# HKPolyU-UAV/ReinforcementLearningPlatform

Hardware: NVIDIA B200
Metric: env-steps/sec (higher is better)
Workload: dtype f64

## Files before the change

### reinforcementlearningplatform_b200/csrc/common.cuh

```cuda
#pragma once
#include <cuda_runtime.h>
#include <stdint.h>
#include <math.h>
#include "../../include/b200env.h"
#include "fastmath64.cuh"

#define B200_BLOCK 128

template <typename T> struct Mth;

template <> struct Mth<double> {
#ifdef B200_LIBDEVICE_MATH
    static __device__ __forceinline__ void sincos(double x, double *s, double *c) { ::sincos(x, s, c); }
    static __device__ __forceinline__ void sincos3(double a, double b, double c, double *sa, double *ca, double *sb,
                                                   double *cb, double *sc, double *cc) {
        ::sincos(a, sa, ca); ::sincos(b, sb, cb); ::sincos(c, sc, cc);
    }
    static __device__ __forceinline__ void sincos2(double a, double b, double *sa, double *ca, double *sb, double *cb) {
        ::sincos(a, sa, ca); ::sincos(b, sb, cb);
    }
    static __device__ __forceinline__ double rcp(double y) { return 1.0 / y; }
    static __device__ __forceinline__ double div(double x, double y) { return x / y; }
    static __device__ __forceinline__ double tanh(double x) { return ::tanh(x); }
    static __device__ __forceinline__ double log(double x) { return ::log(x); }
    static __device__ __forceinline__ double log_nonneg(double x) { return ::log(x); }
    static __device__ __forceinline__ double exp(double x) { return ::exp(x); }
    static __device__ __forceinline__ double asin(double x) { return ::asin(x); }
#else
    static __device__ __forceinline__ void sincos(double x, double *s, double *c) { fm64::sincos(x, s, c); }
    static __device__ __forceinline__ void sincos3(double a, double b, double c, double *sa, double *ca, double *sb,
                                                   double *cb, double *sc, double *cc) {
        fm64::sincos3(a, b, c, sa, ca, sb, cb, sc, cc);
    }
    static __device__ __forceinline__ void sincos2(double a, double b, double *sa, double *ca, double *sb, double *cb) {
        fm64::sincos2(a, b, sa, ca, sb, cb);
    }
    static __device__ __forceinline__ double rcp(double y) { return fm64::rcp(y); }
    static __device__ __forceinline__ double div(double x, double y) { return fm64::div(x, y); }
    static __device__ __forceinline__ double tanh(double x) { return fm64::tanh(x); }
    static __device__ __forceinline__ double log(double x) { return fm64::log(x); }
    static __device__ __forceinline__ double log_nonneg(double x) { return fm64::log_nonneg(x); }
    static __device__ __forceinline__ double exp(double x) { return fm64::exp(x); }
    static __device__ __forceinline__ double asin(double x) { return fm64::asin(x); }
#endif
#ifndef B200_LIBDEVICE_MATH
    static __device__ __forceinline__ double sin(double x) { double s, c; fm64::sincos(x, &s, &c); return s; }
    static __device__ __forceinline__ double cos(double x) { double s, c; fm64::sincos(x, &s, &c); return c; }
#else
    static __device__ __forceinline__ double sin(double x) { return ::sin(x); }
    static __device__ __forceinline__ double cos(double x) { return ::cos(x); }
#endif
    static __device__ __forceinline__ double sin_ld(double x) { return ::sin(x); }
    static __device__ __forceinline__ double tan(double x) { return ::tan(x); }
    static __device__ __forceinline__ double pow(double x, double y) { return ::pow(x, y); }
    static __device__ __forceinline__ double sqrt(double x) { return ::sqrt(x); }
    static __device__ __forceinline__ double acos(double x) { return ::acos(x); }
    static __device__ __forceinline__ double atan2(double y, double x) { return ::atan2(y, x); }
    static __device__ __forceinline__ double abs(double x) { return ::fabs(x); }
    static __device__ __forceinline__ double min(double a, double b) { return ::fmin(a, b); }
    static __device__ __forceinline__ double max(double a, double b) { return ::fmax(a, b); }
    static __device__ __forceinline__ double fma(double a, double b, double c) { return ::fma(a, b, c); }
};

template <> struct Mth<float> {
    static __device__ __forceinline__ float sin(float x) { return ::sinf(x); }
    static __device__ __forceinline__ float sin_ld(float x) { return ::sinf(x); }
    static __device__ __forceinline__ float cos(float x) { return ::cosf(x); }
    static __device__ __forceinline__ void sincos(float x, float *s, float *c) { ::sincosf(x, s, c); }
    static __device__ __forceinline__ void sincos3(float a, float b, float c, float *sa, float *ca, float *sb, float *cb,
                                                   float *sc, float *cc) {
        ::sincosf(a, sa, ca); ::sincosf(b, sb, cb); ::sincosf(c, sc, cc);
    }
    static __device__ __forceinline__ void sincos2(float a, float b, float *sa, float *ca, float *sb, float *cb) {
        ::sincosf(a, sa, ca); ::sincosf(b, sb, cb);
    }
    static __device__ __forceinline__ float rcp(float y) { return 1.0f / y; }
    static __device__ __forceinline__ float div(float x, float y) { return x / y; }
    static __device__ __forceinline__ float tan(float x) { return ::tanf(x); }
    static __device__ __forceinline__ float tanh(float x) { return ::tanhf(x); }
    static __device__ __forceinline__ float pow(float x, float y) { return ::powf(x, y); }
    static __device__ __forceinline__ float log(float x) { return ::logf(x); }
    static __device__ __forceinline__ float log_nonneg(float x) { return ::logf(x); }
    static __device__ __forceinline__ float exp(float x) { return ::expf(x); }
    static __device__ __forceinline__ float sqrt(float x) { return ::sqrtf(x); }
    static __device__ __forceinline__ float asin(float x) { return ::asinf(x); }
    static __device__ __forceinline__ float acos(float x) { return ::acosf(x); }
    static __device__ __forceinline__ float atan2(float y, float x) { return ::atan2f(y, x); }
    static __device__ __forceinline__ float abs(float x) { return ::fabsf(x); }
    static __device__ __forceinline__ float min(float a, float b) { return ::fminf(a, b); }
    static __device__ __forceinline__ float max(float a, float b) { return ::fmaxf(a, b); }
    static __device__ __forceinline__ float fma(float a, float b, float c) { return ::fmaf(a, b, c); }
};

template <typename T>
__device__ __forceinline__ T pow_from_log(T L, T a) {
    const T r = Mth<T>::exp(a * L);
    return a == (T)0 ? (T)1 : r;
}

#ifndef B200_SOA_INDEX
template <typename T, bool IO32, typename I>
__device__ __forceinline__ T ldio(const void *base, I n, int field, I i) {
    constexpr int ES = IO32 ? 4 : (int)sizeof(T);
    const char *p = static_cast<const char *>(base) + (uint64_t)(uint32_t)i * ES + (uint64_t)(uint32_t)n * (uint32_t)(field * ES);
    if (IO32) return (T) * reinterpret_cast<const float *>(p);
    return *reinterpret_cast<const T *>(p);
}
template <typename T, bool IO32, typename I>
__device__ __forceinline__ void stio(void *base, I n, int field, I i, T v) {
    constexpr int ES = IO32 ? 4 : (int)sizeof(T);
    char *p = static_cast<char *>(base) + (uint64_t)(uint32_t)i * ES + (uint64_t)(uint32_t)n * (uint32_t)(field * ES);
    if (IO32) *reinterpret_cast<float *>(p) = (float)v;
    else *reinterpret_cast<T *>(p) = v;
}
#else
template <typename T, bool IO32, typename I>
__device__ __forceinline__ T ldio(const void *base, I n, int field, I i) {
    if (IO32) return (T) static_cast<const float *>(base)[(I)field * n + i];
    return static_cast<const T *>(base)[(I)field * n + i];
}
template <typename T, bool IO32, typename I>
__device__ __forceinline__ void stio(void *base, I n, int field, I i, T v) {
    if (IO32) static_cast<float *>(base)[(I)field * n + i] = (float)v;
    else static_cast<T *>(base)[(I)field * n + i] = v;
}
#endif

template <typename T, bool IO32, typename I>
__device__ __forceinline__ T ldio_idx(const void *base, I n, int field, I i) {
    if (IO32) return (T) static_cast<const float *>(base)[(I)field * n + i];
    return static_cast<const T *>(base)[(I)field * n + i];
}
template <typename T, bool IO32, typename I>
__device__ __forceinline__ void stio_idx(void *base, I n, int field, I i, T v) {
    if (IO32) static_cast<float *>(base)[(I)field * n + i] = (float)v;
    else static_cast<T *>(base)[(I)field * n + i] = v;
}

template <typename T>
__device__ __forceinline__ T np_norm2(T a, T b) { return Mth<T>::sqrt(Mth<T>::fma(b, b, a * a)); }

__device__ __forceinline__ double mul_rn(double a, double b) { return __dmul_rn(a, b); }
__device__ __forceinline__ float mul_rn(float a, float b) { return __fmul_rn(a, b); }
__device__ __forceinline__ double add_rn(double a, double b) { return __dadd_rn(a, b); }
__device__ __forceinline__ float add_rn(float a, float b) { return __fadd_rn(a, b); }
template <typename T>
__device__ __forceinline__ T sumsq_rn(T a, T b) { return add_rn(mul_rn(a, a), mul_rn(b, b)); }
template <typename T>
__device__ __forceinline__ T sumsq_rn(T a, T b, T c, T d) {
    return add_rn(add_rn(sumsq_rn(a, b), mul_rn(c, c)), mul_rn(d, d));
}

template <typename T>
__device__ __forceinline__ T clampc(T x, T lo, T hi) {
    x = x < lo ? lo : x;
    return x > hi ? hi : x;
}

// ... 138 lines not shown
```

### reinforcementlearningplatform_b200/csrc/fastmath64.cuh

```cuda
#pragma once
#include <cuda_runtime.h>
#include <math.h>
#include <math_constants.h>
#include <stdint.h>

namespace fm64 {

static __constant__ double kS[6] = {-0x1.5555555555555p-3, 0x1.1111111110b23p-7, -0x1.a01a019e623afp-13,
                                    0x1.71de376b9c575p-19, -0x1.ae5fdeb852566p-26, 0x1.5dfb4dfaf15abp-33};
static __constant__ double kC[6] = {0x1.5555555555555p-5, -0x1.6c16c16c1691fp-10, 0x1.a01a019f3df42p-16,
                                    -0x1.27e4fa025e03dp-22, 0x1.1eeb52bea9072p-29, -0x1.906dd38cb66a1p-37};
static __constant__ double kE[10] = {0x1.0000000000001p-1, 0x1.5555555555556p-3, 0x1.5555555553b6cp-5,
                                     0x1.1111111110918p-7, 0x1.6c16c1794e1dcp-10, 0x1.a01a01a83ba17p-13,
                                     0x1.a019b621f9d08p-16, 0x1.71de0be2b5e96p-19, 0x1.2894f52583578p-22,
                                     0x1.af3ce42b12b24p-26};
static __constant__ double kL[7] = {0x1.5555555555558p-1, 0x1.99999999949c3p-2, 0x1.2492492ef134dp-2,
                                    0x1.c71c61a265960p-3, 0x1.74630fb47b087p-3, 0x1.39f2ac8e848c3p-3,
                                    0x1.2be78035f90e7p-3};
static __constant__ double kA[12] = {0x1.555555555554fp-3, 0x1.3333333336f25p-4, 0x1.6db6db682abf8p-5,
                                     0x1.f1c71fa66977fp-6, 0x1.6e8b28e7f8608p-6, 0x1.1c596afc9d8acp-6,
                                     0x1.c86de3215c77bp-7, 0x1.8546aebb901aap-7, 0x1.fdf3b5f7fbfb1p-8,
                                     0x1.07d821fcdce60p-6, -0x1.64309bd35e9c9p-7, 0x1.cf09bf99f54b7p-6};
static __constant__ double kR[8] = {0x1.921fb54442d18p+0, 0x1.1a62633145c07p-54, -0x1.f1976b7ed8fbcp-110,
                                    0x1.45f306dc9c883p-1, 0x1.62e42fefa39efp-1, 0x1.abc9e3b39803fp-56,
                                    0x1.71547652b82fep+0, 6755399441055744.0};

__device__ __forceinline__ double rcp(double y) {
    double r;
    asm("rcp.approx.ftz.f64 %0, %1;" : "=d"(r) : "d"(y));
    double e = fma(-y, r, 1.0);
    r = fma(r, e, r);
    e = fma(-y, r, 1.0);
    r = fma(r, e, r);
    return r;
}
__device__ __forceinline__ double div(double x, double y) {
    const double r = rcp(y);
    const double q = x * r;
    return fma(fma(-y, q, x), r, q);
}

__device__ __forceinline__ double sqrt_nb(double x) {
    double y;
    asm("rsqrt.approx.ftz.f64 %0, %1;" : "=d"(y) : "d"(x));
    double g = x * y, h = 0.5 * y;
    double r = fma(-g, h, 0.5);
    g = fma(g, r, g);
    h = fma(h, r, h);
    r = fma(-g, h, 0.5);
    g = fma(g, r, g);
    h = fma(h, r, h);
    g = fma(fma(-g, g, x), h, g);
    return (x == 0.0 || x == CUDART_INF) ? x : g;
}

__device__ __forceinline__ void sincos_core(double x, double *sn, double *cs) {
    const double t = fma(x, kR[3], kR[7]);
    const int n = __double2loint(t);
    const double fn = t - kR[7];
    double r = fma(-fn, kR[0], x);
    r = fma(-fn, kR[1], r);
    r = fma(-fn, kR[2], r);
    const double z = r * r;
    double ps = kS[5];
    ps = fma(ps, z, kS[4]); ps = fma(ps, z, kS[3]); ps = fma(ps, z, kS[2]); ps = fma(ps, z, kS[1]); ps = fma(ps, z, kS[0]);
    ps = fma(r * z, ps, r);
    double pc = kC[5];
    pc = fma(pc, z, kC[4]); pc = fma(pc, z, kC[3]); pc = fma(pc, z, kC[2]); pc = fma(pc, z, kC[1]); pc = fma(pc, z, kC[0]);
    pc = fma(z, fma(z, pc, -0.5), 1.0);
    const double s = (n & 1) ? pc : ps;
    const double c = (n & 1) ? ps : pc;
    *sn = __hiloint2double(__double2hiint(s) ^ ((n & 2) << 30), __double2loint(s));
    *cs = __hiloint2double(__double2hiint(c) ^ (((n + 1) & 2) << 30), __double2loint(c));
}

__device__ __forceinline__ void sincos(double x, double *sn, double *cs) {
    if (!(fabs(x) < 1.0e5)) {
        ::sincos(x, sn, cs);
        return;
    }
    sincos_core(x, sn, cs);
}

__device__ __forceinline__ void sincos3(double a, double b, double c, double *sa, double *ca, double *sb, double *cb,
                                        double *sc, double *cc) {
    if (!(fabs(a) + fabs(b) + fabs(c) < 1.0e5)) {
        ::sincos(a, sa, ca);
        ::sincos(b, sb, cb);
        ::sincos(c, sc, cc);
        return;
    }
    sincos_core(a, sa, ca);
    sincos_core(b, sb, cb);
    sincos_core(c, sc, cc);
}
__device__ __forceinline__ void sincos2(double a, double b, double *sa, double *ca, double *sb, double *cb) {
    if (!(fabs(a) + fabs(b) < 1.0e5)) {
        ::sincos(a, sa, ca);
        ::sincos(b, sb, cb);
        return;
    }
    sincos_core(a, sa, ca);
    sincos_core(b, sb, cb);
}

__device__ __forceinline__ double exp_core(double x) {
    const double t = fma(x, kR[6], kR[7]);
    const int n = __double2loint(t);
    const double fn = t - kR[7];
    double r = fma(-fn, kR[4], x);
    r = fma(-fn, kR[5], r);
    const double r2 = r * r;
    double pe = kE[8], po = kE[9];
    pe = fma(pe, r2, kE[6]); po = fma(po, r2, kE[7]);
    pe = fma(pe, r2, kE[4]); po = fma(po, r2, kE[5]);
    pe = fma(pe, r2, kE[2]); po = fma(po, r2, kE[3]);
    pe = fma(pe, r2, kE[0]); po = fma(po, r2, kE[1]);
    const double p = fma(po, r, pe);
    const double y = fma(r2, p, r) + 1.0;
    return y * __hiloint2double((n + 1023) << 20, 0);
}

__device__ __forceinline__ double exp(double x) {
    double y = exp_core(x);
    if (x < -708.0) y = 0.0;
    if (x > 709.0) y = CUDART_INF;
    return y;
}

__device__ __forceinline__ double log(double x) {
    int hi = __double2hiint(x);
    const int lo = __double2loint(x);
    int k = (hi >> 20) - 1023;
    hi &= 0x000fffff;
    const int i = (hi + 0x95f64) & 0x100000;
    k += i >> 20;
    const double m = __hiloint2double(hi | (i ^ 0x3ff00000), lo);
    const double f = m - 1.0;
    const double s = div(f, 2.0 + f);
    const double z = s * s;
    double R = kL[6];
    R = fma(R, z, kL[5]); R = fma(R, z, kL[4]); R = fma(R, z, kL[3]); R = fma(R, z, kL[2]); R = fma(R, z, kL[1]);
    R = fma(R, z, kL[0]);
    R *= z;
    const double hfsq = 0.5 * f * f;
    const double dk = (double)k;
    double y = dk * kR[4] - ((hfsq - (s * (hfsq + R) + dk * kR[5])) - f);
    if (x < 2.2250738585072014e-308) y = -CUDART_INF;
    if (!(x >= 0.0)) y = CUDART_NAN;
    if (x == CUDART_INF) y = x;
    return y;
}

__device__ __forceinline__ double log_nonneg(double x) {
    int hi = __double2hiint(x);
    const int lo = __double2loint(x);
    int k = (hi >> 20) - 1023;
    hi &= 0x000fffff;
    const int i = (hi + 0x95f64) & 0x100000;
    k += i >> 20;
    const double m = __hiloint2double(hi | (i ^ 0x3ff00000), lo);
    const double f = m - 1.0;
    const double s = div(f, 2.0 + f);
    const double z = s * s;
    double R = kL[6];
    R = fma(R, z, kL[5]); R = fma(R, z, kL[4]); R = fma(R, z, kL[3]); R = fma(R, z, kL[2]); R = fma(R, z, kL[1]);
    R = fma(R, z, kL[0]);
    R *= z;
    const double hfsq = 0.5 * f * f;
    const double dk = (double)k;
    const double y = dk * kR[4] - ((hfsq - (s * (hfsq + R) + dk * kR[5])) - f);
    return x < 2.2250738585072014e-308 ? -CUDART_INF : y;
}

__device__ __forceinline__ double tanh(double x) {
    const double ax = (fabs(x) > 20.0) ? 20.0 : fabs(x);
    const double t = exp_core(2.0 * ax);
    const double y = fma(-2.0, rcp(t + 1.0), 1.0);
    return copysign(y, x);
}

__device__ __forceinline__ double asin(double x) {
    const double ax = fabs(x);
    const bool big = ax > 0.5;
    const double w = big ? 0.5 * (1.0 - ax) : ax * ax;
    const double t = big ? sqrt_nb(w) : ax;
// ... 11 lines not shown
```

### reinforcementlearningplatform_b200/csrc/uav.cu

```cuda
#include "common.cuh"
#ifndef UAV_POS_MINBLOCKS
#define UAV_POS_MINBLOCKS 4
#endif
#ifndef UAV_ATT_MINBLOCKS
#define UAV_ATT_MINBLOCKS 5
#endif
#include "uav_common.cuh"

namespace {
using namespace uavk;

template <typename T>
__device__ __forceinline__ int terminal_flag(const P &p, const T *x, double time) {
    int flag = 0;
    bool out = false;
#pragma unroll
    for (int i = 0; i < 3; ++i) out = out || (x[i] < (T)p.pos_lo[i]) || (x[i] > (T)p.pos_hi[i]);
    if (out) flag = 2;
    out = false;
#pragma unroll
    for (int i = 0; i < 3; ++i) out = out || (x[6 + i] < (T)p.att_lo[i]) || (x[6 + i] > (T)p.att_hi[i]);
    if (out) flag = 3;
    if (time > p.t_term) flag = 1;
    return flag;
// ... 156 lines not shown
    }
}

template <typename T, bool IO32>
__global__ void __launch_bounds__(B200_BLOCK)
uav_att_reset_kernel(const __grid_constant__ P p, const __grid_constant__ b200env_io io, int64_t n,
                     const uint8_t *mask, uint64_t seed, int64_t off, int observe_only) {
    const int64_t i = (int64_t)blockIdx.x * blockDim.x + threadIdx.x;
    if (i >= n) return;
    if (!observe_only && mask && !mask[i]) return;
    T x[12];
    if (observe_only) {
#pragma unroll
        for (int k = 0; k < 6; ++k) { x[k] = (T)0; x[6 + k] = UAV_LDS(io.state, n, k, i); }
    } else {
        att_reset_state<T, int64_t>(p, io, n, i, seed, off, x);
    }
    if (io.next_obs) {
        T ref[3], dref[3], o[6];
#pragma unroll
        for (int k = 0; k < 3; ++k) { ref[k] = UAV_LDS(io.state, n, A_REF + k, i); dref[k] = UAV_LDS(io.state, n, A_DREF + k, i); }
        Trig<T> t;
        t.eval(x[6], x[7], x[8], false);
        att_observe<T>(x, t, ref, dref, o);
#pragma unroll
        for (int k = 0; k < 6; ++k) stio<T, IO32>(io.next_obs, n, k, i, o[k]);
    }
}

enum { P_SIG = 12, P_S1 = 15, P_AREF = 18, P_K1 = 21, P_K2 = 24, P_GAM = 27, P_LMD = 30, P_AMP = 33, P_PER = 37,
       P_PHS = 41, P_PREF = 45, P_DPREF = 48, P_NEXT_PQR0 = 51  };

template <typename T, typename I>
__device__ __forceinline__ void pos_reset_state(const P &p, const b200env_io &io, I n, I i, uint64_t seed,
                                               int64_t off, T *x) {
    const uint32_t ep = io.episode[i];
#pragma unroll
    for (int k = 0; k < 12; ++k) { x[k] = (T)p.init_state[k]; UAV_STS(io.state, n, k, i, x[k]); }
#pragma unroll
    for (int k = 0; k < 3; ++k) {
        UAV_STS(io.state, n, P_SIG + k, i, (T)0);
        UAV_STS(io.state, n, P_S1 + k, i, (T)0);
        UAV_STS(io.state, n, P_K1 + k, i, (T)p.pos_k1[k]);
        UAV_STS(io.state, n, P_K2 + k, i, (T)p.pos_k2[k]);
        UAV_STS(io.state, n, P_GAM + k, i, (T)p.pos_gamma[k]);
        UAV_STS(io.state, n, P_LMD + k, i, (T)p.pos_lmd[k]);
    }
    double A[4], Tp[4], ph[4];
    Philox rng(seed, (uint64_t)(off + (int64_t)i), ep);
    if (p.random_trajectory) {
        const double a = rng.uniform(0., p.traj_A_hi[0]);
        const double tt = rng.uniform(p.traj_T_lo, p.traj_T_hi);
        A[0] = A[1] = A[2] = a; A[3] = 0.;
#pragma unroll
        for (int k = 0; k < 4; ++k) { Tp[k] = tt; ph[k] = p.ref_bias_phase[k]; }
    } else {
#pragma unroll
        for (int k = 0; k < 4; ++k) { A[k] = p.ref_amplitude[k]; Tp[k] = p.ref_period[k]; ph[k] = p.ref_bias_phase[k]; }
    }
    if (p.yaw_fixed) { A[3] = 0.; ph[3] = 0.; }
#pragma unroll
    for (int k = 0; k < 4; ++k) {
        UAV_STS(io.state, n, P_AMP + k, i, (T)A[k]);
        UAV_STS(io.state, n, P_PER + k, i, (T)Tp[k]);
        UAV_STS(io.state, n, P_PHS + k, i, (T)ph[k]);
    }
    if (p.random_pos0) {
#pragma unroll
        for (int k = 0; k < 3; ++k) {
            const double t0 = p.ref_bias_a[k] + A[k] * ::sin(ph[k]);
            const double r = ::fabs(p.init_pos_r[k]);
            const double pos0 = rng.uniform(t0 - r, t0 + r);
            x[k] = (T)pos0;
            x[9 + k] = UAV_LDS(io.state, n, P_NEXT_PQR0 + k, i);
            UAV_STS(io.state, n, k, i, x[k]);
            UAV_STS(io.state, n, 9 + k, i, x[9 + k]);
            UAV_STS(io.state, n, P_NEXT_PQR0 + k, i, x[k]);
        }
    }
    io.time[i] = 0.0;
    io.episode[i] = ep + 1u;
}

template <typename T, typename I, bool IO32>
__device__ __forceinline__ void uav_pos_step_one(const P &p, const Consts<T> &c, const b200env_io &io, I n, I i,
                                                 uint32_t flags, uint64_t seed, int64_t off) {
    T x[12];
#pragma unroll
    for (int k = 0; k < 12; ++k) x[k] = UAV_LDS(io.state, n, k, i);
    double time = io.time[i];
    T a[8], dis[3] = {(T)0, (T)0, (T)0};
#pragma unroll
    for (int k = 0; k < 8; ++k) a[k] = ldio<T, IO32>(io.action, n, k, i);
    if (io.dis) {
#pragma unroll
        for (int k = 0; k < 3; ++k) dis[k] = ldio<T, IO32>(io.dis, n, k, i);
    }
    T sig[3], s1[3], aref0, aref1, rA[4], rT[4], rP[4];
#pragma unroll
    for (int k = 0; k < 3; ++k) { sig[k] = UAV_LDS(io.state, n, P_SIG + k, i); s1[k] = UAV_LDS(io.state, n, P_S1 + k, i); }
    aref0 = UAV_LDS(io.state, n, P_AREF + 0, i);
    aref1 = UAV_LDS(io.state, n, P_AREF + 1, i);
#pragma unroll
    for (int k = 0; k < 4; ++k) {
        rA[k] = UAV_LDS(io.state, n, P_AMP + k, i); rT[k] = UAV_LDS(io.state, n, P_PER + k, i); rP[k] = UAV_LDS(io.state, n, P_PHS + k, i);
    }
    T k1[3], k2[3], gam[3], lmd[3];
#pragma unroll
    for (int k = 0; k < 3; ++k) {
        k1[k] = a[k] > (T)0 ? a[k] : UAV_LDS(io.state, n, P_K1 + k, i);
        k2[k] = a[k + 3] > (T)0 ? a[k + 3] : UAV_LDS(io.state, n, P_K2 + k, i);
        gam[k] = a[6] > (T)0 ? a[6] : UAV_LDS(io.state, n, P_GAM + k, i);
        lmd[k] = a[7] > (T)0 ? a[7] : UAV_LDS(io.state, n, P_LMD + k, i);
        UAV_STS(io.state, n, P_K1 + k, i, k1[k]);
        UAV_STS(io.state, n, P_K2 + k, i, k2[k]);
        UAV_STS(io.state, n, P_GAM + k, i, gam[k]);
        UAV_STS(io.state, n, P_LMD + k, i, lmd[k]);
    }
    T ref[4], dref[4], ddref[4];
    {
        const T bias4[4] = {(T)p.ref_bias_a[0], (T)p.ref_bias_a[1], (T)p.ref_bias_a[2], (T)p.ref_bias_a[3]};
        ref_channels<T, 4>((T)time, rA, rT, bias4, rP, ref, dref, ddref);
    }
    T ctrl[3];
    const T kt_m = c.kt_m;
#pragma unroll
    for (int k = 0; k < 3; ++k) {
        const T e = x[k] - ref[k], de = x[3 + k] - dref[k];
        T so, dso1, pa1_de;
        smc_axis<T>(e, de, k1[k], gam[k], (T)p.pos_alpha[k], (T)p.pos_beta[k], lmd[k], c.dt, sig[k], so, dso1, pa1_de);
        UAV_STS(io.state, n, P_SIG + k, i, sig[k]);
        const T uo1 = kt_m * x[3 + k] + ddref[k] - k1[k] * de - pa1_de - lmd[k] * dso1;
        const T uo2 = -k2[k] * so;
        ctrl[k] = uo1 + uo2;
    }
    const T u_acc = -(ctrl[0] * ctrl[0] * (T)p.R[0] + ctrl[1] * ctrl[1] * (T)p.R[1] + ctrl[2] * ctrl[2] * (T)p.R[2]);
    Trig<T> t1;
    t1.eval(x[6], x[7], x[8], true);
    const T uf = (ctrl[2] + c.g) * c.m / (t1.cphi * t1.cth);
    const T asin_phi_d = clampc<T>(Mth<T>::div((ctrl[0] * t1.spsi - ctrl[1] * t1.cpsi) * c.m, uf), (T)-1, (T)1);
    T phi_d = Mth<T>::asin(asin_phi_d);
    const T asin_theta_d = clampc<T>(
        Mth<T>::div((ctrl[0] * t1.cpsi + ctrl[1] * t1.spsi) * c.m, uf * cos_of_asin<T>(asin_phi_d, phi_d)), (T)-1, (T)1);
    T theta_d = Mth<T>::asin(asin_theta_d);
    const T lim = (T)p.att_limit;
    phi_d = clampc<T>(phi_d, -lim, lim);
    theta_d = clampc<T>(theta_d, -lim, lim);
    T rho_d[3] = {phi_d, theta_d, ref[3]};
#ifdef B200_STRICT_DIV
    T drho_d[3] = {(phi_d - aref0) / c.dt, (theta_d - aref1) / c.dt, dref[3]};
#else
    const Divisor<T> by_dt(c.dt);
    T drho_d[3] = {by_dt.div(phi_d - aref0), by_dt.div(theta_d - aref1), dref[3]};
#endif
    const T rl = (T)p.dot_att_ref_limit;
#pragma unroll
    for (int k = 0; k < 3; ++k) {
        drho_d[k] = clampc<T>(drho_d[k], -rl, rl);
        rho_d[k] = rho_d[k] + drho_d[k] * c.dt;
        UAV_STS(io.state, n, P_AREF + k, i, rho_d[k]);
    }
    T torque[3], d1[3], ak1[3], ak2[3], agam[3], almd[3], aalpha[3], abeta[3];
#pragma unroll
    for (int k = 0; k < 3; ++k) {
        ak1[k] = (T)p.att_k1[k]; ak2[k] = (T)p.att_k2[k]; agam[k] = (T)p.att_gamma[k]; almd[k] = (T)p.att_lmd[k];
        aalpha[k] = (T)p.att_alpha[k]; abeta[k] = (T)p.att_beta[k];
    }
    att_control<T>(c, x, t1, ak1, ak2, agam, almd, aalpha, abeta, s1, rho_d, drho_d, torque, d1);
#pragma unroll
    for (int k = 0; k < 3; ++k) UAV_STS(io.state, n, P_S1 + k, i, s1[k]);
    if (io.obs) {
#pragma unroll
        for (int k = 0; k < 3; ++k) {
            stio<T, IO32>(io.obs, n, k, i, x[k] - ref[k]);
            stio<T, IO32>(io.obs, n, 3 + k, i, x[3 + k] - dref[k]);
        }
    }
    uav_rk44<T, false>(c, x, t1, uf, torque, dis);
    time += p.dt;
    const int flag = terminal_flag<T>(p, x, time);
    const bool done = flag != 0;
    T nxt[6];
#pragma unroll
    for (int k = 0; k < 3; ++k) { nxt[k] = x[k] - ref[k]; nxt[3 + k] = x[3 + k] - dref[k]; }
    const T u_pos = -(nxt[0] * nxt[0] * (T)p.Q_e[0] + nxt[1] * nxt[1] * (T)p.Q_e[1] + nxt[2] * nxt[2] * (T)p.Q_e[2]);
    const T u_vel = -(nxt[3] * nxt[3] * (T)p.Q_de[0] + nxt[4] * nxt[4] * (T)p.Q_de[1] + nxt[5] * nxt[5] * (T)p.Q_de[2]);
    T u_extra = (T)0;
    if (flag == 2 || flag == 3) {
        const T nn = (T)((p.time_max - time) / p.dt);
        u_extra = nn * (u_pos + u_vel + u_acc);
    }
    const T reward = u_pos + u_vel + u_acc + u_extra;
#pragma unroll
    for (int k = 0; k < 6; ++k) stio<T, IO32>(io.next_obs, n, k, i, nxt[k]);
    stio<T, IO32>(io.reward, n, 0, i, reward);
    io.done[i] = done ? 1 : 0;
    io.flag[i] = flag;
    if (done && (flags & B200ENV_AUTO_RESET)) {
        T xr[12];
        pos_reset_state<T, I>(p, io, n, i, seed, off, xr);
#pragma unroll
        for (int k = 0; k < 3; ++k) { nxt[k] = xr[k] - ref[k]; nxt[3 + k] = xr[3 + k] - dref[k]; }
    } else {
#pragma unroll
        for (int k = 0; k < 12; ++k) UAV_STS(io.state, n, k, i, x[k]);
        io.time[i] = time;
        if (done) {
#pragma unroll
            for (int k = 0; k < 3; ++k) { UAV_STS(io.state, n, P_PREF + k, i, ref[k]); UAV_STS(io.state, n, P_DPREF + k, i, dref[k]); }
        }
    }
    if (io.reset_obs) {
#pragma unroll
        for (int k = 0; k < 6; ++k) stio<T, IO32>(io.reset_obs, n, k, i, nxt[k]);
    }
}

template <typename T, typename I, bool IO32>
__global__ void __launch_bounds__(B200_BLOCK, UAV_POS_MINBLOCKS)
uav_pos_step_kernel(const __grid_constant__ P p, const __grid_constant__ UavDerived dv,
                    const __grid_constant__ b200env_io io, int64_t n_, uint32_t flags, uint64_t seed, int64_t off) {
    const int64_t gi = (int64_t)blockIdx.x * blockDim.x + threadIdx.x;
    if (gi >= n_) return;
    const Consts<T> c(p.m, p.g, p.J, p.kr, p.kt, p.dt, dv);
    uav_pos_step_one<T, I, IO32>(p, c, io, (I)n_, (I)gi, flags, seed, off);
}

template <typename T, bool IO32>
__global__ void __launch_bounds__(B200_BLOCK)
uav_pos_reset_kernel(const __grid_constant__ P p, const __grid_constant__ b200env_io io, int64_t n,
                     const uint8_t *mask, uint64_t seed, int64_t off, int observe_only) {
    const int64_t i = (int64_t)blockIdx.x * blockDim.x + threadIdx.x;
    if (i >= n) return;
    if (!observe_only && mask && !mask[i]) return;
    T x[12];
    if (observe_only) {
#pragma unroll
        for (int k = 0; k < 12; ++k) x[k] = UAV_LDS(io.state, n, k, i);
    } else {
        pos_reset_state<T, int64_t>(p, io, n, i, seed, off, x);
    }
    if (io.next_obs) {
#pragma unroll
        for (int k = 0; k < 3; ++k) {
            stio<T, IO32>(io.next_obs, n, k, i, x[k] - UAV_LDS(io.state, n, P_PREF + k, i));
            stio<T, IO32>(io.next_obs, n, 3 + k, i, x[3 + k] - UAV_LDS(io.state, n, P_DPREF + k, i));
        }
    }
}

}

#define UAV_LAUNCH(kern, ...) B200_LAUNCH_TIO(kern, b200_grid(n), B200_BLOCK, s, __VA_ARGS__)

#define UAV_LAUNCH_STEP(kern, fields, gridexpr, ...)                                                                        \
    do {                                                                                                           \
        const bool i32 = (int64_t)(fields) * n < ((int64_t)1 << 32);                                               \
        const bool o32 = b200_io32(io);                                                                            \
        const unsigned g = (gridexpr);                                                                             \
        if (dtype == B200ENV_F64) {                                                                                \
            if (i32 && o32) kern<double, uint32_t, true><<<g, B200_BLOCK, 0, s>>>(__VA_ARGS__);                    \
            else if (i32) kern<double, uint32_t, false><<<g, B200_BLOCK, 0, s>>>(__VA_ARGS__);                     \
            else if (o32) kern<double, int64_t, true><<<g, B200_BLOCK, 0, s>>>(__VA_ARGS__);                       \
            else kern<double, int64_t, false><<<g, B200_BLOCK, 0, s>>>(__VA_ARGS__);                               \
        } else {                                                                                                   \
            if (i32) kern<float, uint32_t, false><<<g, B200_BLOCK, 0, s>>>(__VA_ARGS__);                           \
            else kern<float, int64_t, false><<<g, B200_BLOCK, 0, s>>>(__VA_ARGS__);                                \
        }                                                                                                          \
    } while (0)

int uav_att_dims(int variant, int *sf, int *od, int *ad, int *dd) {
    if (variant != 0) return B200ENV_EENV;
    if (sf) *sf = B200_UAV_ATT_STATE_FIELDS;
    if (od) *od = 6;
    if (ad) *ad = 8;
    if (dd) *dd = 0;
    return B200ENV_OK;
}
int uav_pos_dims(int variant, int *sf, int *od, int *ad, int *dd) {
    if (variant != 0 && variant != 1) return B200ENV_EENV;
    if (sf) *sf = variant == 1 ? B200_UAV_POS_STATE_FIELDS_V1 : B200_UAV_POS_STATE_FIELDS;
    if (od) *od = 6;
    if (ad) *ad = 8;
    if (dd) *dd = 3;
    return B200ENV_OK;
}

static int uav_check_step(const b200env_io *io, uint32_t flags) {
    if (!io->state || !io->time || !io->action || !io->next_obs || !io->reward || !io->done || !io->flag) return B200ENV_ENULL;
    if ((flags & B200ENV_AUTO_RESET) && !io->episode) return B200ENV_ENULL;
    return B200ENV_OK;
}

int uav_att_step(int dtype, int64_t n, const void *params, const b200env_io *io, uint32_t flags, uint64_t seed,
                 int64_t off, cudaStream_t s) {
    int rc = uav_check_step(io, flags);
    if (rc) return rc;
    const P &p = *static_cast<const P *>(params);
    UAV_LAUNCH_STEP(uav_att_step_kernel, B200_UAV_ATT_STATE_FIELDS, b200_grid(n), p, uav_derive(p.m, p.J, p.kt), *io, n, flags, seed, off);
    return b200_check_launch();
}
int uav_pos_step(int dtype, int64_t n, const void *params, const b200env_io *io, uint32_t flags, uint64_t seed,
                 int64_t off, cudaStream_t s) {
    int rc = uav_check_step(io, flags);
    if (rc) return rc;
    const P &p = *static_cast<const P *>(params);
    UAV_LAUNCH_STEP(uav_pos_step_kernel, B200_UAV_POS_STATE_FIELDS_V1, b200_grid(n), p, uav_derive(p.m, p.J, p.kt), *io, n, flags, seed, off);
    return b200_check_launch();
// ... 28 lines not shown
```

### reinforcementlearningplatform_b200/csrc/uav_common.cuh

```cuda
#pragma once
#include "common.cuh"

#ifdef B200_STRICT
#define B200_STRICT_POW
#define B200_STRICT_TAN
#define B200_STRICT_DIV
#ifndef B200_UAV_LAPACK_INV
#define B200_UAV_LAPACK_INV
#endif
#endif
#ifdef B200_STRICT_DIV
#define UAV_DIV(a, b, rb) ((a) / (b))
#else
#define UAV_DIV(a, b, rb) ((a) * (rb))
#endif

template <typename T, typename I>
__device__ __forceinline__ const char *uav_blk_base(const void *base, I i) {
    return static_cast<const char *>(base) +
           (uint64_t)((uint32_t)i >> 7) * (uint64_t)(B200_UAV_STATE_SLOTS * 128 * sizeof(T)) +
           ((uint32_t)i & 127u) * (uint32_t)sizeof(T);
}
#define UAV_LDS(base, n, field, i) (*reinterpret_cast<const T *>(uav_blk_base<T>(base, i) + (field) * (int)(128 * sizeof(T))))
#define UAV_STS(base, n, field, i, v) (*reinterpret_cast<T *>(const_cast<char *>(uav_blk_base<T>(base, i)) + (field) * (int)(128 * sizeof(T))) = (v))

namespace uavk {

typedef b200_uav_params P;



template <typename T>
struct Trig {
    T sphi, cphi, sth, cth, spsi, cpsi, tth, rcth;
    __device__ __forceinline__ void eval(T phi, T th, T psi, bool need_psi) {
        if (need_psi) {
            Mth<T>::sincos3(phi, th, psi, &sphi, &cphi, &sth, &cth, &spsi, &cpsi);
        } else {
            Mth<T>::sincos2(phi, th, &sphi, &cphi, &sth, &cth);
            spsi = (T)0; cpsi = (T)1;
        }
        rcth = Mth<T>::rcp(cth);
#ifdef B200_STRICT_TAN
        tth = Mth<T>::tan(th);
#else
        tth = sth * rcth;
#endif
    }
};

struct UavDerived {
    double rJ[3], rm, kt_m, J21, J02, J10;
};
static inline UavDerived uav_derive(double m, const double *J, double kt) {
    UavDerived d;
    for (int k = 0; k < 3; ++k) d.rJ[k] = 1.0 / J[k];
    d.rm = 1.0 / m;
    d.kt_m = kt / m;
    d.J21 = J[2] - J[1]; d.J02 = J[0] - J[2]; d.J10 = J[1] - J[0];
    return d;
}

template <typename T>
struct Consts {
    T m, g, kr, kt, J0, J1, J2, J21, J02, J10, dt, rJ0, rJ1, rJ2, rm, kt_m;
    __device__ __forceinline__ Consts(double m_, double g_, const double *J, double kr_, double kt_, double dt_,
                                      const UavDerived &d)
        : m((T)m_), g((T)g_), kr((T)kr_), kt((T)kt_), J0((T)J[0]), J1((T)J[1]), J2((T)J[2]), J21((T)d.J21),
          J02((T)d.J02), J10((T)d.J10), dt((T)dt_), rJ0((T)d.rJ[0]), rJ1((T)d.rJ[1]), rJ2((T)d.rJ[2]), rm((T)d.rm),
          kt_m((T)d.kt_m) {}
};

template <typename T, bool ATT_ONLY>
__device__ __forceinline__ void uav_ode(const Consts<T> &c, const T *x, const Trig<T> &t, T throttle, const T *tq,
                                        const T *dis, T *d) {
    const T p = x[9], q = x[10], r = x[11];
    d[9] = UAV_DIV(-c.kr * p - q * r * c.J21 + tq[0], c.J0, c.rJ0);
    d[10] = UAV_DIV(-c.kr * q - p * r * c.J02 + tq[1], c.J1, c.rJ1);
    d[11] = UAV_DIV(-c.kr * r - p * q * c.J10 + tq[2], c.J2, c.rJ2);
    d[6] = p + (t.tth * t.sphi) * q + (t.tth * t.cphi) * r;
    d[7] = t.cphi * q - t.sphi * r;
    d[8] = UAV_DIV(t.sphi, t.cth, t.rcth) * q + UAV_DIV(t.cphi, t.cth, t.rcth) * r;
    if (!ATT_ONLY) {
        d[0] = x[3]; d[1] = x[4]; d[2] = x[5];
        d[3] = UAV_DIV(throttle * (t.cpsi * t.sth * t.cphi + t.spsi * t.sphi) - c.kt * x[3] + dis[0], c.m, c.rm);
        d[4] = UAV_DIV(throttle * (t.spsi * t.sth * t.cphi - t.cpsi * t.sphi) - c.kt * x[4] + dis[1], c.m, c.rm);
        d[5] = -c.g + UAV_DIV(throttle * t.cphi * t.cth - c.kt * x[5] + dis[2], c.m, c.rm);
    }
}

template <typename T, bool ATT_ONLY>
__device__ __forceinline__ void uav_rk44(const Consts<T> &c, T *x, Trig<T> t, T throttle, const T *tq, const T *dis) {
    constexpr int LO = ATT_ONLY ? 6 : 0;
    const T h = c.dt;
    T acc[12], xs[12];
#pragma unroll
    for (int i = LO; i < 12; ++i) { acc[i] = (T)0; xs[i] = x[i]; }
#pragma unroll 1
    for (int s = 0; s < 4; ++s) {
        T d[12];
        uav_ode<T, ATT_ONLY>(c, xs, t, throttle, tq, dis, d);
        const T w = (s == 0 || s == 3) ? (T)1 : (T)2;
        const T cs = (s == 2) ? (T)1 : (T)0.5;
#pragma unroll
        for (int i = LO; i < 12; ++i) {
            const T k = h * d[i];
            acc[i] = acc[i] + w * k;
            xs[i] = x[i] + k * cs;
        }
        if (s < 3) t.eval(xs[6], xs[7], xs[8], !ATT_ONLY);
    }
#pragma unroll
    for (int i = LO; i < 12; ++i) x[i] = x[i] + UAV_DIV(acc[i], (T)6, (T)(1.0 / 6.0));
    if (x[8] > (T)M_PI) x[8] -= (T)(2 * M_PI);
    if (x[8] < (T)-M_PI) x[8] += (T)(2 * M_PI);
}

template <typename T>
__device__ __forceinline__ void smc_axis(T e, T de, T k1, T gamma, T alpha, T beta, T lmd, T dt, T &integ,
                                         T &s_out, T &dot_s1, T &pa1_de) {
    const T ae = Mth<T>::abs(e);
#ifdef B200_STRICT_POW
    const T s_ = de + k1 * e + gamma * Mth<T>::pow(ae, alpha) * Mth<T>::tanh((T)5 * e);
    dot_s1 = Mth<T>::pow(Mth<T>::abs(s_), beta) * Mth<T>::tanh((T)5 * s_);
    integ += dot_s1 * dt;
    s_out = s_ + lmd * integ;
    pa1_de = gamma * alpha * Mth<T>::pow(ae, alpha - (T)1) * de;
    return;
#endif
    const T L = Mth<T>::log_nonneg(ae);
    const T pa1 = pow_from_log<T>(L, alpha - (T)1);
    const T pa_ = pa1 * ae;
    const T pa = alpha == (T)0 ? (T)1 : ((ae == (T)0 && alpha > (T)0) ? (T)0 : pa_);
    const T s = de + k1 * e + gamma * pa * Mth<T>::tanh((T)5 * e);
    dot_s1 = pow_from_log<T>(Mth<T>::log_nonneg(Mth<T>::abs(s)), beta) * Mth<T>::tanh((T)5 * s);
    integ += dot_s1 * dt;
    s_out = s + lmd * integ;
    pa1_de = gamma * alpha * pa1 * de;
}

template <typename T>
__device__ __forceinline__ void neg_inv_apply(T b00, T b01, T b02, T b11, T b12, T b21, T b22, const T *v, T *out) {
    const bool swap = Mth<T>::abs(b21) > Mth<T>::abs(b11);
    const T u11 = swap ? b21 : b11, u12 = swap ? b22 : b12;
    const T r21 = swap ? b11 : b21, r22 = swap ? b12 : b22;
    const T l = r21 * ((T)1 / u11);
    const T u22 = r22 - l * u12;
    T inv[3][3];
#pragma unroll
    for (int cidx = 0; cidx < 3; ++cidx) {
        T y0 = cidx == 0 ? (T)1 : (T)0;
        T y1 = (cidx == (swap ? 2 : 1)) ? (T)1 : (T)0;
        T y2 = (cidx == (swap ? 1 : 2)) ? (T)1 : (T)0;
        y2 = y2 - l * y1;
        const T x2 = y2 / u22;
        const T x1 = (y1 - u12 * x2) / u11;
        const T x0 = ((y0 - b01 * x1) - b02 * x2) / b00;
        inv[0][cidx] = x0; inv[1][cidx] = x1; inv[2][cidx] = x2;
    }
#pragma unroll
    for (int i = 0; i < 3; ++i) out[i] = -(inv[i][0] * v[0] + inv[i][1] * v[1] + inv[i][2] * v[2]);
}

template <typename T>
__device__ __forceinline__ void att_control(const Consts<T> &c, const T *x, const Trig<T> &t, const T *k1, const T *k2,
                                            const T *gamma, const T *lmd, const T *alpha, const T *beta, T *s1,
                                            const T *ref, const T *dref, T *torque, T *d1) {
    const T p = x[9], q = x[10], r = x[11];
    const T f01 = t.sphi * t.tth, f02 = t.cphi * t.tth, f11 = t.cphi, f12 = -t.sphi;
    const T f21 = UAV_DIV(t.sphi, t.cth, t.rcth), f22 = UAV_DIV(t.cphi, t.cth, t.rcth);
    d1[0] = p + f01 * q + f02 * r;
    d1[1] = f11 * q + f12 * r;
    d1[2] = f21 * q + f22 * r;
    const T rc2 = t.rcth * t.rcth;
    const T c2 = t.cth * t.cth;
    (void)c2;
    const T F01 = d1[0] * t.tth * t.cphi + UAV_DIV(d1[1] * t.sphi, c2, rc2);
    const T F02 = -d1[0] * t.tth * t.sphi + UAV_DIV(d1[1] * t.cphi, c2, rc2);
    const T F11 = -d1[0] * t.sphi, F12 = -d1[0] * t.cphi;
    const T F21 = UAV_DIV(d1[0] * t.cphi * t.cth + d1[1] * t.sphi * t.sth, c2, rc2);
    const T F22 = UAV_DIV(-d1[0] * t.sphi * t.cth + d1[1] * t.cphi * t.sth, c2, rc2);
    const T g0 = UAV_DIV(c.kr * p + q * r * (c.J1 - c.J2), c.J0, c.rJ0);
    const T g1 = UAV_DIV(c.kr * q + p * r * (c.J2 - c.J0), c.J1, c.rJ1);
    const T g2 = UAV_DIV(c.kr * r + p * q * (c.J0 - c.J1), c.J2, c.rJ2);
    T sec[3];
    sec[0] = (F01 * q + F02 * r) + (g0 + f01 * g1 + f02 * g2);
    sec[1] = (F11 * q + F12 * r) + (f11 * g1 + f12 * g2);
    sec[2] = (F21 * q + F22 * r) + (f21 * g1 + f22 * g2);
    T v[3];
#pragma unroll
    for (int i = 0; i < 3; ++i) {
        const T e = x[6 + i] - ref[i], de = d1[i] - dref[i];
        T sigma, dot_s1, pa1_de;
        smc_axis<T>(e, de, k1[i], gamma[i], alpha[i], beta[i], lmd[i], c.dt, s1[i], sigma, dot_s1, pa1_de);
        const T u1 = sec[i] + k1[i] * de + pa1_de + lmd[i] * dot_s1;
        const T u2 = -k2[i] * Mth<T>::tanh((T)10 * sigma);
        v[i] = u1 + u2;
    }
#ifdef B200_UAV_LAPACK_INV
    neg_inv_apply<T>(c.rJ0, f01 * c.rJ1, f02 * c.rJ2, f11 * c.rJ1, f12 * c.rJ2, f21 * c.rJ1, f22 * c.rJ2, v, torque);
#else
    torque[0] = -c.J0 * (v[0] - t.sth * v[2]);
    torque[1] = -c.J1 * (t.cphi * v[1] + t.sphi * t.cth * v[2]);
    torque[2] = -c.J2 * (t.cphi * t.cth * v[2] - t.sphi * v[1]);
#endif
}


template <typename T>
__device__ __forceinline__ T cos_of_asin(T u, T phi_d) {
    if (sizeof(T) == 4) return Mth<T>::sqrt(Mth<T>::max(Mth<T>::fma(-u, u, (T)1), (T)0));
    T sn, cs;
    Mth<T>::sincos(phi_d, &sn, &cs);
    return cs;
}

template <typename T, int NCH>
__device__ __forceinline__ void ref_channels(T time, const T *A, const T *period, const T *bias, const T *phase, T *r,
                                             T *dr, T *ddr) {
    T w = (T)0, s = (T)0, co = (T)1;
#pragma unroll
    for (int k = 0; k < NCH; ++k) {
        if (k == 0 || period[k] != period[k - 1] || phase[k] != phase[k - 1]) {
            if (k == 0 || period[k] != period[k - 1]) w = Mth<T>::div((T)(2 * M_PI), period[k]);
            Mth<T>::sincos(w * time + phase[k], &s, &co);
        }
        r[k] = A[k] * s + bias[k];
        dr[k] = A[k] * w * co;
        ddr[k] = -A[k] * (w * w) * s;
    }
}


}
```

Before: 5.583 billion.

## Speculate UAV step with unguarded sincos and fall back to exact path

The UAV position step now runs first with sincos variants that skip the large-argument range-reduction guard and only accumulate a flag when any argument is out of range. If the flag is set, the step restores the saved controller integrator state from shared memory and reruns the step through a noinline guarded path. The aim is to drop the guard and slow-path branches from the hot loop. The cost is extra shared memory, extra register pressure, and a duplicated rare path.

```diff
diff --git a/reinforcementlearningplatform_b200/csrc/common.cuh b/reinforcementlearningplatform_b200/csrc/common.cuh
--- a/reinforcementlearningplatform_b200/csrc/common.cuh
+++ b/reinforcementlearningplatform_b200/csrc/common.cuh
@@ -17,6 +17,16 @@
         ::sincos(a, sa, ca); ::sincos(b, sb, cb); ::sincos(c, sc, cc);
     }
     static __device__ __forceinline__ void sincos2(double a, double b, double *sa, double *ca, double *sb, double *cb) {
+        ::sincos(a, sa, ca); ::sincos(b, sb, cb);
+    }
+    static constexpr bool kNbFlags = false;
+    static __device__ __forceinline__ void sincos_nb(double x, double *s, double *c, bool &) { ::sincos(x, s, c); }
+    static __device__ __forceinline__ void sincos3_nb(double a, double b, double c, double *sa, double *ca, double *sb,
+                                                      double *cb, double *sc, double *cc, bool &) {
+        ::sincos(a, sa, ca); ::sincos(b, sb, cb); ::sincos(c, sc, cc);
+    }
+    static __device__ __forceinline__ void sincos2_nb(double a, double b, double *sa, double *ca, double *sb, double *cb,
+                                                      bool &) {
         ::sincos(a, sa, ca); ::sincos(b, sb, cb);
     }
     static __device__ __forceinline__ double rcp(double y) { return 1.0 / y; }
@@ -34,6 +44,18 @@
     }
     static __device__ __forceinline__ void sincos2(double a, double b, double *sa, double *ca, double *sb, double *cb) {
         fm64::sincos2(a, b, sa, ca, sb, cb);
+    }
+    static constexpr bool kNbFlags = true;
+    static __device__ __forceinline__ void sincos_nb(double x, double *s, double *c, bool &wild) {
+        fm64::sincos_nb(x, s, c, wild);
+    }
+    static __device__ __forceinline__ void sincos3_nb(double a, double b, double c, double *sa, double *ca, double *sb,
+                                                      double *cb, double *sc, double *cc, bool &wild) {
+        fm64::sincos3_nb(a, b, c, sa, ca, sb, cb, sc, cc, wild);
+    }
+    static __device__ __forceinline__ void sincos2_nb(double a, double b, double *sa, double *ca, double *sb, double *cb,
+                                                      bool &wild) {
+        fm64::sincos2_nb(a, b, sa, ca, sb, cb, wild);
     }
     static __device__ __forceinline__ double rcp(double y) { return fm64::rcp(y); }
     static __device__ __forceinline__ double div(double x, double y) { return fm64::div(x, y); }
@@ -74,6 +96,15 @@
     static __device__ __forceinline__ void sincos2(float a, float b, float *sa, float *ca, float *sb, float *cb) {
         ::sincosf(a, sa, ca); ::sincosf(b, sb, cb);
     }
+    static constexpr bool kNbFlags = false;
+    static __device__ __forceinline__ void sincos_nb(float x, float *s, float *c, bool &) { ::sincosf(x, s, c); }
+    static __device__ __forceinline__ void sincos3_nb(float a, float b, float c, float *sa, float *ca, float *sb, float *cb,
+                                                      float *sc, float *cc, bool &) {
+        ::sincosf(a, sa, ca); ::sincosf(b, sb, cb); ::sincosf(c, sc, cc);
+    }
+    static __device__ __forceinline__ void sincos2_nb(float a, float b, float *sa, float *ca, float *sb, float *cb, bool &) {
+        ::sincosf(a, sa, ca); ::sincosf(b, sb, cb);
+    }
     static __device__ __forceinline__ float rcp(float y) { return 1.0f / y; }
     static __device__ __forceinline__ float div(float x, float y) { return x / y; }
     static __device__ __forceinline__ float tan(float x) { return ::tanf(x); }
diff --git a/reinforcementlearningplatform_b200/csrc/fastmath64.cuh b/reinforcementlearningplatform_b200/csrc/fastmath64.cuh
--- a/reinforcementlearningplatform_b200/csrc/fastmath64.cuh
+++ b/reinforcementlearningplatform_b200/csrc/fastmath64.cuh
@@ -102,6 +102,24 @@
     }
     sincos_core(a, sa, ca);
     sincos_core(b, sb, cb);
+}
+
+__device__ __forceinline__ void sincos_nb(double x, double *sn, double *cs, bool &wild) {
+    wild |= !(fabs(x) < 1.0e5);
+    sincos_core(x, sn, cs);
+}
+__device__ __forceinline__ void sincos2_nb(double a, double b, double *sa, double *ca, double *sb, double *cb,
+                                           bool &wild) {
+    wild |= !(fabs(a) + fabs(b) < 1.0e5);
+    sincos_core(a, sa, ca);
+    sincos_core(b, sb, cb);
+}
+__device__ __forceinline__ void sincos3_nb(double a, double b, double c, double *sa, double *ca, double *sb,
+                                           double *cb, double *sc, double *cc, bool &wild) {
+    wild |= !(fabs(a) + fabs(b) + fabs(c) < 1.0e5);
+    sincos_core(a, sa, ca);
+    sincos_core(b, sb, cb);
+    sincos_core(c, sc, cc);
 }
 
 __device__ __forceinline__ double exp_core(double x) {
diff --git a/reinforcementlearningplatform_b200/csrc/uav.cu b/reinforcementlearningplatform_b200/csrc/uav.cu
--- a/reinforcementlearningplatform_b200/csrc/uav.cu
+++ b/reinforcementlearningplatform_b200/csrc/uav.cu
@@ -262,9 +262,11 @@
     io.episode[i] = ep + 1u;
 }
 
-template <typename T, typename I, bool IO32>
-__device__ __forceinline__ void uav_pos_step_one(const P &p, const Consts<T> &c, const b200env_io &io, I n, I i,
+template <typename T, typename I, bool IO32, bool GUARDED>
+__device__ __forceinline__ bool uav_pos_step_one(const P &p, const Consts<T> &c, const b200env_io &io, I n, I i,
                                                  uint32_t flags, uint64_t seed, int64_t off) {
+    constexpr bool CHECK = !GUARDED && Mth<T>::kNbFlags;
+    bool wild = false;
     T x[12];
 #pragma unroll
     for (int k = 0; k < 12; ++k) x[k] = UAV_LDS(io.state, n, k, i);
@@ -281,6 +283,13 @@
     for (int k = 0; k < 3; ++k) { sig[k] = UAV_LDS(io.state, n, P_SIG + k, i); s1[k] = UAV_LDS(io.state, n, P_S1 + k, i); }
     aref0 = UAV_LDS(io.state, n, P_AREF + 0, i);
     aref1 = UAV_LDS(io.state, n, P_AREF + 1, i);
+    __shared__ T saved[8][B200_BLOCK];
+    if (CHECK) {
+#pragma unroll
+        for (int k = 0; k < 3; ++k) { saved[k][threadIdx.x] = sig[k]; saved[3 + k][threadIdx.x] = s1[k]; }
+        saved[6][threadIdx.x] = aref0;
+        saved[7][threadIdx.x] = aref1;
+    }
 #pragma unroll
     for (int k = 0; k < 4; ++k) {
         rA[k] = UAV_LDS(io.state, n, P_AMP + k, i); rT[k] = UAV_LDS(io.state, n, P_PER + k, i); rP[k] = UAV_LDS(io.state, n, P_PHS + k, i);
@@ -300,7 +309,7 @@
     T ref[4], dref[4], ddref[4];
     {
         const T bias4[4] = {(T)p.ref_bias_a[0], (T)p.ref_bias_a[1], (T)p.ref_bias_a[2], (T)p.ref_bias_a[3]};
-        ref_channels<T, 4>((T)time, rA, rT, bias4, rP, ref, dref, ddref);
+        wild |= ref_channels<T, 4, GUARDED>((T)time, rA, rT, bias4, rP, ref, dref, ddref);
     }
     T ctrl[3];
     const T kt_m = c.kt_m;
@@ -316,12 +325,12 @@
     }
     const T u_acc = -(ctrl[0] * ctrl[0] * (T)p.R[0] + ctrl[1] * ctrl[1] * (T)p.R[1] + ctrl[2] * ctrl[2] * (T)p.R[2]);
     Trig<T> t1;
-    t1.eval(x[6], x[7], x[8], true);
+    wild |= t1.template eval<GUARDED>(x[6], x[7], x[8], true);
     const T uf = (ctrl[2] + c.g) * c.m / (t1.cphi * t1.cth);
     const T asin_phi_d = clampc<T>(Mth<T>::div((ctrl[0] * t1.spsi - ctrl[1] * t1.cpsi) * c.m, uf), (T)-1, (T)1);
     T phi_d = Mth<T>::asin(asin_phi_d);
     const T asin_theta_d = clampc<T>(
-        Mth<T>::div((ctrl[0] * t1.cpsi + ctrl[1] * t1.spsi) * c.m, uf * cos_of_asin<T>(asin_phi_d, phi_d)), (T)-1, (T)1);
+        Mth<T>::div((ctrl[0] * t1.cpsi + ctrl[1] * t1.spsi) * c.m, uf * cos_of_asin<T, GUARDED>(asin_phi_d, phi_d, wild)), (T)-1, (T)1);
     T theta_d = Mth<T>::asin(asin_theta_d);
     const T lim = (T)p.att_limit;
     phi_d = clampc<T>(phi_d, -lim, lim);
@@ -356,7 +365,18 @@
             stio<T, IO32>(io.obs, n, 3 + k, i, x[3 + k] - dref[k]);
         }
     }
-    uav_rk44<T, false>(c, x, t1, uf, torque, dis);
+    wild |= uav_rk44<T, false, GUARDED>(c, x, t1, uf, torque, dis);
+    if (CHECK && wild) {
+        volatile T (*sv)[B200_BLOCK] = saved;
+#pragma unroll
+        for (int k = 0; k < 3; ++k) {
+            UAV_STS(io.state, n, P_SIG + k, i, sv[k][threadIdx.x]);
+            UAV_STS(io.state, n, P_S1 + k, i, sv[3 + k][threadIdx.x]);
+        }
+        UAV_STS(io.state, n, P_AREF + 0, i, sv[6][threadIdx.x]);
+        UAV_STS(io.state, n, P_AREF + 1, i, sv[7][threadIdx.x]);
+        return false;
+    }
     time += p.dt;
     const int flag = terminal_flag<T>(p, x, time);
     const bool done = flag != 0;
@@ -394,6 +414,14 @@
 #pragma unroll
         for (int k = 0; k < 6; ++k) stio<T, IO32>(io.reset_obs, n, k, i, nxt[k]);
     }
+    return true;
+}
+
+template <typename T, typename I, bool IO32>
+__device__ __noinline__ void uav_pos_step_exact(const P &p, const UavDerived &dv, const b200env_io &io, I n, I i,
+                                                uint32_t flags, uint64_t seed, int64_t off) {
+    const Consts<T> c(p.m, p.g, p.J, p.kr, p.kt, p.dt, dv);
+    uav_pos_step_one<T, I, IO32, true>(p, c, io, n, i, flags, seed, off);
 }
 
 template <typename T, typename I, bool IO32>
@@ -403,7 +431,8 @@
     const int64_t gi = (int64_t)blockIdx.x * blockDim.x + threadIdx.x;
     if (gi >= n_) return;
     const Consts<T> c(p.m, p.g, p.J, p.kr, p.kt, p.dt, dv);
-    uav_pos_step_one<T, I, IO32>(p, c, io, (I)n_, (I)gi, flags, seed, off);
+    if (!uav_pos_step_one<T, I, IO32, false>(p, c, io, (I)n_, (I)gi, flags, seed, off))
+        uav_pos_step_exact<T, I, IO32>(p, dv, io, (I)n_, (I)gi, flags, seed, off);
 }
 
 template <typename T, bool IO32>
diff --git a/reinforcementlearningplatform_b200/csrc/uav_common.cuh b/reinforcementlearningplatform_b200/csrc/uav_common.cuh
--- a/reinforcementlearningplatform_b200/csrc/uav_common.cuh
+++ b/reinforcementlearningplatform_b200/csrc/uav_common.cuh
@@ -33,11 +33,15 @@
 template <typename T>
 struct Trig {
     T sphi, cphi, sth, cth, spsi, cpsi, tth, rcth;
-    __device__ __forceinline__ void eval(T phi, T th, T psi, bool need_psi) {
+    template <bool GUARDED = true>
+    __device__ __forceinline__ bool eval(T phi, T th, T psi, bool need_psi) {
+        bool wild = false;
         if (need_psi) {
-            Mth<T>::sincos3(phi, th, psi, &sphi, &cphi, &sth, &cth, &spsi, &cpsi);
+            if (GUARDED) Mth<T>::sincos3(phi, th, psi, &sphi, &cphi, &sth, &cth, &spsi, &cpsi);
+            else Mth<T>::sincos3_nb(phi, th, psi, &sphi, &cphi, &sth, &cth, &spsi, &cpsi, wild);
         } else {
-            Mth<T>::sincos2(phi, th, &sphi, &cphi, &sth, &cth);
+            if (GUARDED) Mth<T>::sincos2(phi, th, &sphi, &cphi, &sth, &cth);
+            else Mth<T>::sincos2_nb(phi, th, &sphi, &cphi, &sth, &cth, wild);
             spsi = (T)0; cpsi = (T)1;
         }
         rcth = Mth<T>::rcp(cth);
@@ -46,6 +50,7 @@
 #else
         tth = sth * rcth;
 #endif
+        return wild;
     }
 };
 
@@ -89,11 +94,12 @@
     }
 }
 
-template <typename T, bool ATT_ONLY>
-__device__ __forceinline__ void uav_rk44(const Consts<T> &c, T *x, Trig<T> t, T throttle, const T *tq, const T *dis) {
+template <typename T, bool ATT_ONLY, bool GUARDED = true>
+__device__ __forceinline__ bool uav_rk44(const Consts<T> &c, T *x, Trig<T> t, T throttle, const T *tq, const T *dis) {
     constexpr int LO = ATT_ONLY ? 6 : 0;
     const T h = c.dt;
     T acc[12], xs[12];
+    bool wild = false;
 #pragma unroll
     for (int i = LO; i < 12; ++i) { acc[i] = (T)0; xs[i] = x[i]; }
 #pragma unroll 1
@@ -108,12 +114,13 @@
             acc[i] = acc[i] + w * k;
             xs[i] = x[i] + k * cs;
         }
-        if (s < 3) t.eval(xs[6], xs[7], xs[8], !ATT_ONLY);
+        if (s < 3) wild |= t.template eval<GUARDED>(xs[6], xs[7], xs[8], !ATT_ONLY);
     }
 #pragma unroll
     for (int i = LO; i < 12; ++i) x[i] = x[i] + UAV_DIV(acc[i], (T)6, (T)(1.0 / 6.0));
     if (x[8] > (T)M_PI) x[8] -= (T)(2 * M_PI);
     if (x[8] < (T)-M_PI) x[8] += (T)(2 * M_PI);
+    return wild;
 }
 
 template <typename T>
@@ -207,29 +214,38 @@
 }
 
 
-template <typename T>
-__device__ __forceinline__ T cos_of_asin(T u, T phi_d) {
+template <typename T, bool GUARDED = true>
+__device__ __forceinline__ T cos_of_asin(T u, T phi_d, bool &wild) {
     if (sizeof(T) == 4) return Mth<T>::sqrt(Mth<T>::max(Mth<T>::fma(-u, u, (T)1), (T)0));
     T sn, cs;
-    Mth<T>::sincos(phi_d, &sn, &cs);
+    if (GUARDED) Mth<T>::sincos(phi_d, &sn, &cs);
+    else Mth<T>::sincos_nb(phi_d, &sn, &cs, wild);
     return cs;
 }
-
-template <typename T, int NCH>
-__device__ __forceinline__ void ref_channels(T time, const T *A, const T *period, const T *bias, const T *phase, T *r,
+template <typename T>
+__device__ __forceinline__ T cos_of_asin(T u, T phi_d) {
+    bool unused = false;
+    return cos_of_asin<T, true>(u, phi_d, unused);
+}
+
+template <typename T, int NCH, bool GUARDED = true>
+__device__ __forceinline__ bool ref_channels(T time, const T *A, const T *period, const T *bias, const T *phase, T *r,
                                              T *dr, T *ddr) {
     T w = (T)0, s = (T)0, co = (T)1;
+    bool wild = false;
 #pragma unroll
     for (int k = 0; k < NCH; ++k) {
         if (k == 0 || period[k] != period[k - 1] || phase[k] != phase[k - 1]) {
             if (k == 0 || period[k] != period[k - 1]) w = Mth<T>::div((T)(2 * M_PI), period[k]);
-            Mth<T>::sincos(w * time + phase[k], &s, &co);
+            if (GUARDED) Mth<T>::sincos(w * time + phase[k], &s, &co);
+            else Mth<T>::sincos_nb(w * time + phase[k], &s, &co, wild);
         }
         r[k] = A[k] * s + bias[k];
         dr[k] = A[k] * w * co;
         ddr[k] = -A[k] * (w * w) * s;
     }
-}
-
-
-}
+    return wild;
+}
+
+
+}
```

Result: no change. 5.620 billion, median of 6 (+0.7%).
